# marsermd/DeepestScatter

Measured on AMD Instinct MI355X. Metric: Msamples/s (rays x spp) at 512^3 vol, 1024^2 frame; HBM GB/s vs roofline, higher is better.
Workload: dtype f32

## Files before the change

### deepestscatter_amd/cloudtrace.py

```python
from __future__ import annotations

import ctypes as C
from dataclasses import dataclass
from pathlib import Path

import numpy as np

from . import _lib
from ._lib import (CT_BUF_DENSITY, CT_BUF_FRAME, CT_BUF_INSCATTER, CT_BUF_M2, CT_BUF_MEAN, CT_BUF_SCREEN,
                   CtCounters, CtFetchCounters, CtScene, check)

MIE_FILE = Path(__file__).resolve().parent / "data" / "mie_raw.f32"

LIGHT_DIRECTIONS = {
    "Front": (-0.586, -0.766, -0.271),
    "Side": (-0.03, -0.25, 0.8),
    "Back": (0.586, -0.766, -0.271),
}


def load_mie_raw() -> tuple[np.ndarray, np.ndarray]:
    raw = np.fromfile(MIE_FILE, dtype="<f4")
    if raw.size != 8192:
        raise RuntimeError(f"{MIE_FILE} is corrupt")
# ... 545 lines not shown
        c = CtCounters()
        check(self.L.ct_counters(self.h, C.byref(c)), self.h)
        return c.as_dict()

    def fetch_counters(self) -> dict:
        c = CtFetchCounters()
        check(self.L.ct_fetch_counters(self.h, C.byref(c)), self.h)
        return c.as_dict()

    def debug_invariants(self) -> dict:
        out = np.zeros(8, np.uint64)
        check(self.L.ct_debug_invariants(self.h, _p(out)), self.h)
        names = ["armed", "checks", "violations", "samples_without_alpha_1", "dealt", "resumed", "written", "suspended"]
        return {n: int(v) for n, v in zip(names, out)}

    def debug_memory(self) -> dict:
        out = np.zeros(8, np.uint64)
        check(self.L.ct_debug_memory(self.h, _p(out)), self.h)
        names = ["raw_texture", "density_bricks", "inscatter_bricks", "march_bricks_dense", "march_bricks_stored", "sparse",
                 "row_table", "coarse_clearance"]
        return {n: int(v) for n, v in zip(names, out)}

    def delta_grid(self) -> dict:
        out = np.zeros(8, np.uint32)
        check(self.L.ct_debug_delta_grid(self.h, _p(out)), self.h)
        return {"cell": int(out[0]), "stored": tuple(int(v) for v in out[1:4]), "origin": tuple(int(v) for v in out[4:7]),
                "nee": int(out[7] & 0xff), "interior": bool(out[7] & 0x100)}

    def march_meta(self) -> dict:
        geom = np.zeros(8, np.uint32)
        check(self.L.ct_debug_march_meta(self.h, _p(geom), C.c_void_p(), 0), self.h)
        d = {"radius": int(geom[0]), "bias_x": int(geom[1]), "bias": int(geom[2]),
             "bricks": tuple(int(v) for v in geom[3:6]), "sparse": bool(geom[6]), "meta": None}
        if not d["sparse"]:
            gx, gy, gz = d["bricks"]
            meta = np.zeros((gz * 4, gy * 4, gx), np.uint8)
            check(self.L.ct_debug_march_meta(self.h, _p(geom), _p(meta), meta.size), self.h)
            d["meta"] = meta
        return d

    LAYOUTS = ("density_bricks", "shadow_bricks", "march_bricks", "march_rows", "march_coarse", "twin_bricks", "majorant_cells",
               "majorant_codes", "mip_pyramid")

    def layout(self, which) -> tuple[np.ndarray, dict]:
        which = self.LAYOUTS.index(which) if isinstance(which, str) else int(which)
        geom, n = np.zeros(16, np.uint32), C.c_size_t(0)
        check(self.L.ct_debug_layout(self.h, which, _p(geom), C.c_void_p(), 0, C.byref(n)), self.h)
        g = [int(v) for v in geom]
        raw = np.zeros(n.value, np.uint8)
        check(self.L.ct_debug_layout(self.h, which, _p(geom), _p(raw), raw.size, C.byref(n)), self.h)
        if which in (_lib.CT_LAYOUT_DENSITY_BRICKS, _lib.CT_LAYOUT_SHADOW_BRICKS, _lib.CT_LAYOUT_TWIN_BRICKS):
            d = {"bias": g[0], "bricks": tuple(g[1:4])}
            return raw.reshape(g[3], g[2], g[1], 128), d
        if which == _lib.CT_LAYOUT_MARCH_BRICKS:
            d = {"bias_x": g[0], "bias": g[1], "bricks": tuple(g[2:5]), "sparse": bool(g[5])}
            return (raw.reshape(-1, 128) if d["sparse"] else raw.reshape(g[4], g[3], g[2], 128)), d
        if which == _lib.CT_LAYOUT_MARCH_ROWS:
            return raw.view(np.uint32).reshape(g[1], g[0], 2), {"rows": (g[0], g[1])}
        if which == _lib.CT_LAYOUT_MARCH_COARSE:
            return raw.reshape(g[3], g[2], g[1]), {"shift": g[0], "cells": tuple(g[1:4]), "bias": g[4]}
        if which == _lib.CT_LAYOUT_MIP_PYRAMID:
            return raw, {"levels": g[0], "dims": tuple(g[1:4])}
        d = {"cell": g[0], "div": g[1], "stored": tuple(g[2:5]), "origin": tuple(g[5:8]), "virtual": tuple(g[8:11]), "bias": g[11]}
        return raw.reshape(g[4], g[3], g[2]), d

    def kernel_time(self):
        a, b, n = C.c_double(0), C.c_double(0), C.c_uint64(0)
        check(self.L.ct_kernel_time(self.h, C.byref(a), C.byref(b), C.byref(n)), self.h)
        return float(a.value), float(b.value), int(n.value)

    def set_stream(self, hip_stream: int | None):
        check(self.L.ct_set_stream(self.h, C.c_void_p(hip_stream) if hip_stream else None), self.h)

    def debug_stats(self) -> dict:
        out = np.zeros(64, np.uint64)
        check(self.L.ct_debug_stats(self.h, _p(out)), self.h)
        names = ["regen_phases", "regen_lanes", "march_phases", "march_lanes", "scatter_phases", "scatter_lanes",
                 "fetched_steps", "fetched_zero_cells", "skipped_steps", "zero_cells_nonfree_brick",
                 "zero_cells_free_brick_d1", "skip_loop_wave_iterations", "nee_footprints_reused", "waves",
                 "stolen_jobs", "max_scheduler_visits_of_a_wave"]
        d = {n: int(v) for n, v in zip(names, out)}
        d["wave_end_hist_5ms"] = [int(v) for v in out[16:40]]
        d["wave_end_minus_drained_hist_0p5ms"] = [int(v) for v in out[40:64]]
        ex = np.zeros(73, np.uint64)
        check(self.L.ct_debug_stats_ex(self.h, _p(ex), 73), self.h)
        d["march_fetch_same_line_as_lanes_previous"] = int(ex[68])
        d["march_fetch_line_shared_with_a_lower_lane"] = int(ex[69])
        d["nee_lookups_skipped_shadow_zero"] = int(ex[72])
        d["raw"] = [int(v) for v in out]
        d["watchdog"] = int(out[63])
        return d

    def debug_suspended(self) -> int:
        n = C.c_uint64(0)
        check(self.L.ct_debug_suspended(self.h, C.byref(n)), self.h)
        return int(n.value)

    def debug_math_selftest(self, which: int) -> dict:
        out = np.zeros(3, np.uint64)
        check(self.L.ct_debug_math_selftest(self.h, which, _p(out)), self.h)
        return {"tested": int(out[0]), "mismatches": int(out[1]), "first_bad_bits": int(out[2])}

    def debug_cdf_inversion(self, first_u24: int, count: int) -> np.ndarray:
        out = np.empty(count, np.uint32)
        check(self.L.ct_debug_cdf_inversion(self.h, first_u24, count, _p(out)), self.h)
        return out


class TracerGroup:

    def __init__(self, density: np.ndarray, devices, params: SceneParams | None = None, **kw):
        self.L = _lib.load()
        self.params = params or SceneParams(**kw)
        s, keep = make_scene(density, self.params)
        self.width, self.height = self.params.width, self.params.height
        dev = np.asarray(list(devices), np.int32)
        g = C.c_void_p()
        rc = self.L.ct_group_create(C.byref(s), _p(dev), len(dev), C.byref(g))
        del keep
        if rc != _lib.CT_OK:
            msg = self.L.ct_group_last_error(None)
            raise _lib.CloudTraceError(rc, msg.decode("utf-8", "replace") if msg else "")
        self.g = g

    def _check(self, rc):
        if rc != _lib.CT_OK:
            msg = self.L.ct_group_last_error(self.g)
            raise _lib.CloudTraceError(rc, msg.decode("utf-8", "replace") if msg else "")

    def close(self):
        if getattr(self, "g", None):
            for net in list(getattr(self, "_networks", ())):
                net.close()
            self.L.ct_group_destroy(self.g)
            self.g = None

    def __enter__(self):
        return self

    def __exit__(self, *exc):
        self.close()

    def __del__(self):
        try:
            self.close()
        except Exception:
            pass

    def set_camera(self, eye, U, V, W):
        a = [np.asarray(v, np.float32) for v in (eye, U, V, W)]
        self._check(self.L.ct_group_set_camera(self.g, *[_p(v) for v in a]))

    def set_light(self, direction, color=None, intensity: float = 1e6):
        d, c = _light_args(direction, color)
        self._check(self.L.ct_group_set_light(self.g, _p(d) if d is not None else None, _p(c) if c is not None else None, intensity))

    def render_accumulate(self, first_subframe_id: int, count: int):
        self._check(self.L.ct_group_render_accumulate(self.g, first_subframe_id, count))

    def network(self, module_or_weights, width: int | None = None, aux: int | None = None, head_layers: int | None = None):
        return GroupNetwork(self, module_or_weights, width, aux, head_layers)

    def network_render_accumulate(self, net, first_subframe_id: int, count: int, transform="linear", rgb_scale=(1.0, 1.0, 1.0),
                                  band_pixels: int = 0, direct: bool = False):
        p = CloudTracer._network_render_params(transform, rgb_scale, band_pixels, direct)
        self._check(self.L.ct_group_network_render_accumulate(self.g, net.gn if net is not None else None, C.byref(p),
                                                              first_subframe_id & 0xFFFFFFFF, count))

    def reset(self):
        self._check(self.L.ct_group_reset(self.g))

# ... 72 lines not shown
```

### deepestscatter_amd/csrc/ct_api.cpp

```cpp
#include <algorithm>
#include <array>
#include <atomic>
#include <chrono>
#include <climits>
#include <cmath>
#include <cstdarg>
#include <cstdio>
#include <cstdlib>
#include <cstring>
#include <new>
#include <string>
#include <utility>
#include <map>
#include <vector>

#include "../../include/cloudtrace.h"
#include "ct_handle.hpp"

static thread_local std::string g_create_error;

int ct::fail(CtHandle h, int code, const char *fmt, ...)
{
    char buf[512];
    va_list ap;
// ... 436 lines not shown
{
    const uint32_t n[3] = { nx, ny, nz };
    uint32_t faces = 0;
    for (uint32_t f = 0; f < 6; f++) {
        const uint32_t axis = f / 2, u_axis = (axis + 1) % 3, v_axis = (axis + 2) % 3;
        uint32_t c[3];
        c[axis] = (f & 1) ? n[axis] - 1 : 0;
        bool zero = true;
        for (c[v_axis] = 0; zero && c[v_axis] < n[v_axis]; c[v_axis]++) {
            for (c[u_axis] = 0; zero && c[u_axis] < n[u_axis]; c[u_axis]++) {
                zero = t[((size_t)c[2] * ny + c[1]) * nx + c[0]] == 0;
            }
        }
        faces |= (zero ? 1u : 0u) << f;
    }
    return faces;
}

struct MarchStorage {
    bool sparse;
    bool vmm;
    bool pad_rows;
    bool experimental;
};

static MarchStorage march_storage(const CtScene *s, const Knob &sparse_knob)
{
    bool sparse = (s->flags & CT_FLAG_SPARSE_BRICKS) != 0, vmm = (s->flags & CT_FLAG_VMM_BRICKS) != 0, pad_only = false, no_pad = false;
    if (const char *env = sparse_knob.get()) {
        const int v = atoi(env);
        sparse = v == 1;
        vmm = v == 2 || v == 4;
        pad_only = v == 3;
        no_pad = v == 4;
    }
    const bool march = s->estimator == CT_EST_MARCH;
    vmm = vmm && march;
    return { sparse && march, vmm && !sparse, (vmm && !no_pad) || pad_only, vmm || pad_only };
}

static int open_device(const CtScene *s, CtHandle h)
{
    int ndev = 0;
    if (hipGetDeviceCount(&ndev) != hipSuccess || ndev <= 0) {
        return fail(h, CT_E_NODEVICE, "no HIP device visible (libcloudtrace has no CPU fallback)");
    }
    if (s->device < 0 || s->device >= ndev) {
        return fail(h, CT_E_INVAL, "device %d out of range (0..%d)", s->device, ndev - 1);
    }
    HIPCHK(h, hipSetDevice(s->device));
    (void)hipGetLastError();
    HIPCHK(h, hipStreamCreateWithFlags(&h->own_stream, hipStreamNonBlocking));
    h->stream = h->own_stream;
    for (auto &e : h->ev) {
        HIPCHK(h, hipEventCreate(&e));
    }
    return CT_OK;
}

static int choose_schedule(const CtScene *s, CtHandle h)
{
    const CtTuning &t = h->tune;
    DevScene &d = h->dev;
    const bool delta = s->estimator == CT_EST_DELTA, big = beyond_caches(s);
    h->shape = persistent_shape(s->device, delta, knob_int(t.BLOCKS_PER_CU, INT_MIN, INT_MAX, 0));
    h->debug_invariants = knob_flag(t.DEBUG_INVARIANTS, h->debug_invariants);
    h->shape.stats = t.STATS.get() != nullptr || h->debug_invariants;
    h->exchange = delta ? knob_int(t.EXCHANGE, 0, 2, 0) : 0;
#ifdef CT_EXPERIMENTS
    if (h->exchange && (s->flags & CT_FLAG_TEX_FIXED8)) {
        return fail(h, CT_E_INVAL, "CT_EXCHANGE has no CT_FLAG_TEX_FIXED8 kernels");
    }
    if (h->exchange) {
        h->xshape = h->exchange == 2 ? wave_exchange_shape(s->device) : exchange_shape(s->device);
        h->xshape.stats = h->shape.stats;
    }
#else
    if (h->exchange) {
        return fail(h, CT_E_INVAL, "CT_EXCHANGE needs the experiments build (python -m deepestscatter_amd.build --variant exp; "
                                   "CT_LIBRARY=libcloudtrace_exp.so)");
    }
#endif
    d.march_burst = (uint32_t)knob_int(t.MARCH_BURST, 1, 1024, delta ? 2 : 8);
    d.burst_scatter = (uint32_t)knob_int(t.BURST_SCATTER, 1, 65, delta || big ? 48 : 40);
    d.burst_idle = (uint32_t)knob_int(t.BURST_IDLE, 1, 65, 32);
    d.burst_march_min = (uint32_t)knob_int(t.BURST_MARCH_MIN, 1, 64, 1);
    d.tail_burst = (uint32_t)knob_int(t.TAIL_BURST, 1, 1024, 8);
    d.regen_min = (uint32_t)knob_int(t.REGEN_MIN, 1, 64, delta ? 4 : big ? 16 : 8);
    d.scatter_min = (uint32_t)knob_int(t.SCATTER_MIN, 1, 64, delta ? 12 : 1);
    d.scatter_num = 0;
    d.scatter_den = 1;
    if (const char *e = t.SCATTER_RATIO.get()) {
        unsigned a = 1, b = 1;
        if (sscanf(e, "%u/%u", &a, &b) == 2 && b > 0 && a < 1000 && b < 1000) {
            d.scatter_num = a;
            d.scatter_den = b;
        }
    }
    d.hint_period = 64;
    if (const char *e = t.HINT_PERIOD.get()) {
        const int v = atoi(e);
        d.hint_period = (v > 0 && (v & (v - 1)) == 0) ? (uint32_t)v : 0u;
    }
    if (delta) {
        d.delta_nee = (uint32_t)knob_int(t.DELTA_NEE, 0, 2, big ? 2 : 1);
        h->job_work = 48.f;
    }
    h->queues_enabled = knob_flag(t.XCD_QUEUES, big);
    h->regions = (uint32_t)knob_int(t.XCD_REGIONS, 1, 65536, (int)h->regions);
    if (const char *e = t.SHARED_DEPTH.get()) {
        h->shared_depth = (float)atof(e);
    }
    h->job_max = (uint32_t)knob_int(t.JOB_MAX, 1, 4096, (int)h->job_max);
    if (const char *e = t.JOB_WORK.get()) {
        h->job_work = (float)std::max(1.0, atof(e));
    }
    h->no_advance = knob_flag(t.NO_ADVANCE, h->no_advance);
    h->point_order = knob_flag(t.POINT_ORDER, h->point_order);
    h->continuation = knob_flag(t.CONTINUATION, h->continuation) && !h->exchange;
    h->chunk_interleave = knob_flag(t.CHUNK_INTERLEAVE, h->chunk_interleave);
    if (const char *e = t.TILE_ORDER.get()) {
        h->tile_hilbert = strcmp(e, "hilbert") == 0;
    }
    h->chunk_morton = knob_flag(t.CHUNK_MORTON, h->chunk_morton);
    h->serpentine = knob_flag(t.SERPENTINE, h->serpentine);
    h->hand_on_jobs = knob_flag(t.HAND_ON_JOBS, h->hand_on_jobs);
    h->max_age_override = knob_int(t.MAX_AGE, 0, CtHandle_::kMaxRegions - 1, h->max_age_override);
    h->ahead = (uint32_t)knob_int(t.RENDER_AHEAD, 0, 65535, (int)h->ahead);
    return CT_OK;
}

static void light_uniforms(const CtScene *s, DevScene &d)
{
    float l[3] = { s->light_direction[0], s->light_direction[1], s->light_direction[2] };
    if (!(s->flags & CT_FLAG_LIGHT_NORMALIZED)) {
        v3_normalize_twice(s->light_direction, l);
    }
    d.nlx = -l[0];
    d.nly = -l[1];
    d.nlz = -l[2];
    d.lr = s->light_color[0] * s->light_intensity;
    d.lg = s->light_color[1] * s->light_intensity;
    d.lb = s->light_color[2] * s->light_intensity;
}

static void scene_uniforms(const CtScene *s, DevScene &d)
{
    const uint32_t nx = s->dims[0], ny = s->dims[1], nz = s->dims[2];
    const float fx = (float)nx, fy = (float)ny, fz = (float)nz;
    const float maxs = fmaxf(fmaxf(fx, fy), fz);
    d.nx = (int32_t)nx;
    d.ny = (int32_t)ny;
    d.nz = (int32_t)nz;
    d.bx = fx / maxs;
    d.by = fy / maxs;
    d.bz = fz / maxs;
    d.hx = d.bx + 0.01f;
    d.hy = d.by + 0.01f;
    d.hz = d.bz + 0.01f;
    d.tsx = maxs / fx;
    d.tsy = maxs / fy;
    d.tsz = maxs / fz;
    d.sx = (maxs / fx) * fx;
    d.sy = (maxs / fy) * fy;
    d.sz = (maxs / fz) * fz;
    d.density_multiplier = s->cloud_size_m / s->mean_free_path_m;
    d.sample_step = s->sample_step;
// ... 2597 lines not shown
```

### deepestscatter_amd/csrc/ct_internal.hpp

```cpp
#pragma once

#include <hip/hip_runtime.h>
#include <stdint.h>

#include "ct_device.hpp"

namespace ct {

constexpr int kTile = 8;
constexpr int kCounterCount = 9;
constexpr int kStatCount = 73;
constexpr int kContWords = 16;
constexpr int kContWordsDelta = 32;
constexpr int kLeftWords = 8;
constexpr int kQueueFlag = 32;
constexpr int kQueueDone = 16;
constexpr int kQueueWords = 64;
constexpr int kQueues = 8;

struct BatchArgs {
    float4 *frames;
    uint32_t frame_stride;
    const float4 *primary;
    const float4 *advance;
    const uint32_t *pixels;
    const float4 *start;
    const uint32_t *group_rank;
    uint32_t rank_base;
    const uint32_t *job_group;
    const uint32_t *job_sub;
    uint2 *cost;
    uint32_t n_jobs;
    uint32_t q_begin[kQueues + 2];
    uint32_t reverse;
    uint32_t first_subframe;
    uint32_t S;
    uint32_t *queue;
    const uint32_t *cont_in;
    const uint32_t *cont_in_count;
    uint32_t *cont_cursor;
    uint32_t *cont_out;
    uint32_t *cont_out_count;
    uint32_t cont_capacity;
    uint32_t max_age;
    unsigned long long *cont_total;
    const uint32_t *left_in;
    const uint32_t *left_in_count;
    uint32_t *left_cursor;
    uint32_t *left_out;
    uint32_t *left_out_count;
    uint32_t left_capacity;
    uint32_t out_offset;
    unsigned long long *counters;
    unsigned long long *stats;
    unsigned long long *timeline;
    uint32_t *touched_density, *touched_shadow;
};

struct LaunchShape {
    int blocks;
    int threads;
    bool stats;
    uint32_t pool_slots = 0;
    uint32_t scatter_waves = 0;
    bool wide = false;
};

inline void split_queues_evenly(BatchArgs &ba)
{
    for (int x = 0; x <= kQueues; x++) {
        ba.q_begin[x] = (uint32_t)(((uint64_t)ba.n_jobs * (uint32_t)x) / kQueues);
    }
    ba.q_begin[kQueues + 1] = ba.n_jobs;
}

#ifndef CT_SHARD_SHIFT
#define CT_SHARD_SHIFT 0
#endif
__host__ __device__ inline uint32_t tile_owner(uint32_t tx, uint32_t ty, uint32_t shard_count)
{
    return shard_count <= 1 ? 0u : ((tx >> CT_SHARD_SHIFT) + 3u * (ty >> CT_SHARD_SHIFT)) % shard_count;
}

hipError_t launch_build_bricks(const uint8_t *texels, int nx, int ny, int nz, int bias, int gx, int gy, int gz,
                               uint8_t *bricks, hipStream_t stream);
hipError_t launch_build_twin_bricks(const uint8_t *density, const uint8_t *shadow, int nx, int ny, int nz, int bias, int gx, int gy, int gz,
                                    uint8_t *bricks, hipStream_t stream);
hipError_t launch_build_dist(const uint8_t *texels, int nx, int ny, int nz, int bias, int gx, int gy, int gz,
                             uint8_t *dist, uint8_t *scratch, uint8_t *majorant, hipStream_t stream);
hipError_t launch_majorant_cells(const uint8_t *texels, int nx, int ny, int nz, int bias, int cell, const int origin[3], int gx, int gy, int gz,
                                 uint8_t *out, uint8_t *out_codes, hipStream_t stream);
hipError_t launch_brick_meta(const uint8_t *dist, const uint8_t *majorant, int nx, int ny, int nz, int bias, int gx,
                             int gy, int gz, uint8_t *bricks, hipStream_t stream);
hipError_t launch_build_mbricks(const uint8_t *texels, int nx, int ny, int nz, int bias_x, int bias, int gx, int gy,
// ... 148 lines not shown
```

### deepestscatter_amd/csrc/ct_kernels.hip

```cpp
#include <algorithm>
#include <cstdlib>

#include "ct_internal.hpp"

namespace ct {

__global__ void build_bricks_kernel(const uint8_t *__restrict__ t, int nx, int ny, int nz, int bias,
                                    uint8_t *__restrict__ bricks, int gx, int gy, int gz)
{
    const int64_t total = (int64_t)gx * gy * gz * 128;
    for (int64_t i = (int64_t)blockIdx.x * blockDim.x + threadIdx.x; i < total; i += (int64_t)gridDim.x * blockDim.x) {
        const int64_t b = i >> 7;
        const int o = (int)(i & 127);
        uint8_t v = 0;
        if (o < 125) {
            const int lx = o % 5, ly = (o / 5) % 5, lz = o / 25;
            const int x = (int)(b % gx) * 4 + lx - bias;
            const int y = (int)((b / gx) % gy) * 4 + ly - bias;
            const int z = (int)(b / ((int64_t)gx * gy)) * 4 + lz - bias;
            const int xc = min(max(x, 0), nx - 1), yc = min(max(y, 0), ny - 1), zc = min(max(z, 0), nz - 1);
            v = t[((size_t)zc * ny + yc) * nx + xc];
        }
        bricks[i] = v;
    }
// ... 858 lines not shown
                                        uint32_t &nee_key, uint2 &nee_cell, bool &reused, bool zero = false)
{
    NeeLoads n;
    const float cos_light = dot3(mk3(sc.nlx, sc.nly, sc.nlz), dir);
    const float u = (cos_light + 1) / 2;
    const float x = fmaf(u, (float)kMieN, -0.5f);
    const int32_t i = (int32_t)floorf(x);
    const int32_t j = min(max(i, 0), kMieN - 2);
    float2 pair;
#if CT_MARCH_PHASE_LDS == 2
    LdsFloat *table = chopped ? (LdsFloat *)lds.chopped : (LdsFloat *)lds.mie;
    pair = make_float2(table[j], table[j + 1]);
#elif CT_MARCH_PHASE_LDS == 1
    LdsFloat *table = (LdsFloat *)lds.chopped;
    pair = make_float2(table[j], table[j + 1]);
    if (!chopped) {
        GlobalFloat *first = (GlobalFloat *)(sc.mie + j);
        pair = make_float2(first[0], first[1]);
    }
#else
    if (chopped) {
        pair = make_float2(lds.chopped[j], lds.chopped[j + 1]);
    } else {
        __builtin_memcpy(&pair, sc.mie + j, sizeof pair);
    }
#endif
    n.a = (i > kMieN - 2) ? pair.y : pair.x;
    n.b = (i < 0) ? pair.x : pair.y;
    n.w = tex_weight<FIXED8>(x);
    n.cell = fetch_cell_cached<WIDE>(sc, sc.ibricks, pos, nee_key, nee_cell, reused, zero);
    return n;
}

template <bool FIXED8>
CT_DEV f3 in_scattering_finish(const DevScene &sc, const NeeLoads &n, f3 pos)
{
    const float phase = fmaf(n.w, n.b - n.a, n.a);
    const float ins = filter_at<FIXED8>(sc, n.cell, pos);
    f3 l = scale3(mk3(sc.lr, sc.lg, sc.lb), ins);
    l = scale3(l, phase);
    return scale3(l, sc.sun_ratio);
}

enum : int { ST_IDLE = 0, ST_MARCH = 1, ST_BOUNCE = 2 };

#ifndef CT_MARCH_FLAT_ZERO
#define CT_MARCH_FLAT_ZERO 1
#endif
#ifndef CT_MARCH_FLAT_EXIT
#define CT_MARCH_FLAT_EXIT 1
#endif
#ifndef CT_MARCH_FUSE
#define CT_MARCH_FUSE 1
#endif
constexpr bool MARCH_FUSE = CT_MARCH_FUSE != 0;
#ifndef CT_MARCH_NEE_SKIP
#define CT_MARCH_NEE_SKIP 1
#endif

CT_DEV float inv_max_advance(const DevScene &sc, f3 stepv)
{
    const float m = fmaxf(fmaxf(fabsf(stepv.x) * sc.sx, fabsf(stepv.y) * sc.sy), fabsf(stepv.z) * sc.sz);
    return __builtin_amdgcn_rcpf(fmaxf(m, 1e-20f));
}


CT_DEV int skip_steps(uint32_t c, float inv_maxd)
{
    return (int)(((float)c - 0.03125f) * inv_maxd);
}

CT_DEV void replay_steps(f3 &pos, f3 stepv, int n)
{
    int i = 0;
    for (; i + 8 <= n; i += 8) {
#pragma unroll
        for (int k = 0; k < 8; k++) {
            pos = add3(pos, stepv);
        }
    }
    for (; i < n; i++) {
        pos = add3(pos, stepv);
    }
}

template <bool FIXED8, bool SPARSE = false>
__global__ __launch_bounds__(256) void inscatter_kernel(DevScene sc, uint8_t *__restrict__ out, uint32_t zero_faces)
{
    const int64_t total = (int64_t)sc.nx * sc.ny * sc.nz;
    const int64_t i = (int64_t)blockIdx.x * blockDim.x + threadIdx.x;
    if (i >= total) {
        return;
    }
    const int x = (int)(i % sc.nx), y = (int)((i / sc.nx) % sc.ny), z = (int)(i / ((int64_t)sc.nx * sc.ny));
    const float max_size = (float)max(max(sc.nx, sc.ny), sc.nz);
    const float tsx = max_size / (float)sc.nx, tsy = max_size / (float)sc.ny, tsz = max_size / (float)sc.nz;
    const float min_scale = fminf(fminf(tsx, tsy), tsz);
    const float inv_min_scale = 1.0f / min_scale;
    f3 p = mk3((float)x / max_size, (float)y / max_size, (float)z / max_size);
    p = scale3(p, inv_min_scale);
    const f3 step_to_light = scale3(normalize3(mk3(sc.nlx, sc.nly, sc.nlz)), sc.sample_step);
    const int step_count = (int)(1 / sc.sample_step);
    float transmittance = 1;
    int s = 0;
    bool done = false;
    if (sc.mbricks != nullptr && (SPARSE || sc.m_rows == nullptr)) {
        const float inv_maxd = inv_max_advance(sc, step_to_light);
        while (s < step_count && in_box(sc, p)) {
            uint32_t meta;
            const uint2 cell = fetch_cell_m<SPARSE>(sc, p, meta);
            if ((cell.x | cell.y) != 0u) {
                const float density = filter_at<FIXED8>(sc, cell, p) * sc.density_multiplier;
                const float extinction = density * sc.sample_step;
                transmittance *= ct_expf(-extinction);
                if (transmittance * 255.f < 1.f) {
                    done = true;
                    break;
                }
            }
            p = add3(p, step_to_light);
            s += 1;
            const uint32_t clear = meta & 0x3fu;
            if (clear != 0u) {
                const int n = min(skip_steps(clear, inv_maxd), step_count - s);
                replay_steps(p, step_to_light, n);
                s += n;
            }
        }
    }
    for (; !done && s < step_count; s++) {
        const float tx = fmaf(p.x, sc.sx, -0.5f), ty = fmaf(p.y, sc.sy, -0.5f), tz = fmaf(p.z, sc.sz, -0.5f);
        const bool gone = ((zero_faces & 1u) && tx < 0.0f && step_to_light.x <= 0.0f) ||
                          ((zero_faces & 2u) && tx >= (float)(sc.nx - 1) && step_to_light.x >= 0.0f) ||
                          ((zero_faces & 4u) && ty < 0.0f && step_to_light.y <= 0.0f) ||
                          ((zero_faces & 8u) && ty >= (float)(sc.ny - 1) && step_to_light.y >= 0.0f) ||
                          ((zero_faces & 16u) && tz < 0.0f && step_to_light.z <= 0.0f) ||
                          ((zero_faces & 32u) && tz >= (float)(sc.nz - 1) && step_to_light.z >= 0.0f);
        if (gone) {
            break;
        }
        const float density = tex3_clamped<FIXED8>(sc, sc.dbricks, p) * sc.density_multiplier;
        const float extinction = density * sc.sample_step;
        transmittance *= ct_expf(-extinction);
        p = add3(p, step_to_light);
        if (transmittance * 255.f < 1.f) {
            break;
        }
    }
    out[i] = (uint8_t)(transmittance * 255.f);
}

hipError_t launch_inscatter(const DevScene &sc, uint8_t *out, uint32_t zero_faces, hipStream_t stream)
{
    const int64_t total = (int64_t)sc.nx * sc.ny * sc.nz;
    const int threads = 256;
    const int64_t blocks = (total + threads - 1) / threads;
    const dim3 grid((unsigned)blocks), block(threads);
    if (sc.mbricks != nullptr && sc.m_rows != nullptr) {
        if (sc.tex_fixed8) {
            hipLaunchKernelGGL((inscatter_kernel<true, true>), grid, block, 0, stream, sc, out, zero_faces);
        } else {
            hipLaunchKernelGGL((inscatter_kernel<false, true>), grid, block, 0, stream, sc, out, zero_faces);
        }
    } else if (sc.tex_fixed8) {
        hipLaunchKernelGGL(inscatter_kernel<true>, grid, block, 0, stream, sc, out, zero_faces);
    } else {
// ... 42 lines not shown
        }
    }
    advance[p] = make_float4(start.x, start.y, start.z, __uint_as_float(start_bits));
}

hipError_t launch_primary_advance(const DevScene &sc, const float4 *primary, float4 *advance, hipStream_t stream)
{
    const dim3 grid((sc.width + 31) / 32, (sc.height + 7) / 8), block(256);
    if (sc.m_rows) {
        hipLaunchKernelGGL(primary_advance_kernel<true>, grid, block, 0, stream, sc, primary, advance);
    } else {
        hipLaunchKernelGGL(primary_advance_kernel<false>, grid, block, 0, stream, sc, primary, advance);
    }
    return hipGetLastError();
}

__global__ __launch_bounds__(256) void start_records_kernel(DevScene sc, const uint32_t *__restrict__ pixels, uint32_t slots,
                                                            const float4 *__restrict__ primary, const float4 *__restrict__ advance,
                                                            float4 *__restrict__ start)
{
    const uint32_t i = blockIdx.x * 256u + threadIdx.x;
    if (i >= slots) {
        return;
    }
    const uint32_t pixel = pixels[i];
    float4 r0 = make_float4(0.f, 0.f, 0.f, __uint_as_float(0xc0000000u)), r1 = make_float4(0.f, 0.f, 0.f, 0.f);
    if (pixel != 0xffffffffu) {
        const float4 p0 = primary[2 * (size_t)pixel];
        r1 = primary[2 * (size_t)pixel + 1];
        const bool go = p0.w != 0.f && in_box(sc, mk3(p0.x, p0.y, p0.z));
        uint32_t bits = go ? 0u : 0x80000000u;
        r0 = p0;
        if (go && advance) {
            r0 = advance[pixel];
            bits |= __float_as_uint(r0.w) & 0x3fffffffu;
        }
        r0.w = __uint_as_float(bits);
    }
    start[2 * (size_t)i] = r0;
    start[2 * (size_t)i + 1] = r1;
}

hipError_t launch_start_records(const DevScene &sc, const uint32_t *pixels, uint32_t slots, const float4 *primary,
                                const float4 *advance, float4 *start, hipStream_t stream)
{
    hipLaunchKernelGGL(start_records_kernel, dim3((slots + 255u) / 256u), dim3(256), 0, stream, sc, pixels, slots, primary, advance, start);
    return hipGetLastError();
}

template <int MODE, bool STATS, bool SPARSE, bool COST = true, bool FIXED8 = false, bool WIDE = false>
__global__ __launch_bounds__(kMarchThreads) __attribute__((amdgpu_waves_per_eu(6))) void render_persistent_kernel(DevScene sc, BatchArgs ba)
{
    __shared__ MieLdsFull lds;
    load_tables(sc, lds);

    const uint32_t lane = threadIdx.x & 63u;
#ifdef CT_DIAG_TIMELINE
    if (ba.timeline && lane == 0u) {
        ba.timeline[4u * (blockIdx.x * (blockDim.x >> 6) + (threadIdx.x >> 6))] = wall_clock64();
    }
#endif
    f3 pos = mk3(0, 0, 0), dir = mk3(0, 0, 1), stepv = mk3(0, 0, 0), rad = mk3(0, 0, 0);
    uint32_t seed = 0, depth = 0, out_idx = 0;
    uint32_t work = 0;
    float xi = 0, T = 1;
    uint32_t dfree = 0;
    float inv_maxd = 0;
    int state = ST_IDLE;

    JobState job{ 0, 0, 0, 0, 0, 0 };
    bool left_done = false;
    uint32_t q_cur = (uint32_t)kQueues, q_tried = 0;
    bool drained = false;
    uint32_t c_dl = 0, c_il = 0, c_cap = 0;
    uint32_t w_fetch = 0, w_nee = 0;
    uint32_t iv_dealt = 0, iv_written = 0, iv_resumed = 0, iv_suspended = 0;
    uint32_t nee_key = 0xffffffffu;
    uint2 nee_cell = make_uint2(0u, 0u);
    uint32_t st_regen = 0, st_regen_l = 0, st_march = 0, st_march_l = 0, st_scat = 0, st_scat_l = 0;
    uint32_t st_fetch = 0, st_zero = 0, st_skip = 0, st_zero_d0 = 0, st_zero_d1 = 0, st_skip_iters = 0, st_stolen = 0, st_iters = 0, st_first = 0;
    uint32_t st_hit2 = 0, st_hit3 = 0, st_h2 = 0xffffffffu, st_h3 = 0xffffffffu;
    uint32_t st_same_line = 0, st_dup_line = 0, st_prev_line = 0xffffffffu;
    uint32_t st_nee_zero = 0;

    uint32_t age = 0;
    if (ba.cont_in) {
        const uint32_t total = __builtin_amdgcn_readfirstlane(*ba.cont_in_count);
        uint32_t base = 0;
        if (lane == 0) {
            base = atomicAdd(ba.cont_cursor, 64u);
        }
        base = __builtin_amdgcn_readfirstlane(base);
        if (base + lane < total) {
            const uint4 *e = (const uint4 *)(ba.cont_in + (size_t)(base + lane) * kContWords);
            const uint4 w0 = e[0], w1 = e[1], w2 = e[2], w3 = e[3];
            pos = mk3(__uint_as_float(w0.x), __uint_as_float(w0.y), __uint_as_float(w0.z));
            dir = mk3(__uint_as_float(w0.w), __uint_as_float(w1.x), __uint_as_float(w1.y));
            rad = mk3(__uint_as_float(w1.z), __uint_as_float(w1.w), __uint_as_float(w2.x));
            seed = w2.y;
            out_idx = w2.z;
            xi = __uint_as_float(w2.w);
            T = __uint_as_float(w3.x);
            inv_maxd = __uint_as_float(w3.y);
            depth = w3.z & 0xffffu;
            dfree = (w3.z >> 16) & 0xffu;
            state = (int)(w3.z >> 24);
            stepv = scale3(dir, sc.sample_step);
            age = w3.w;
            if (STATS) {
                iv_resumed += 1;
            }
        }
    }
    const bool may_suspend = ba.cont_out != nullptr;
    const bool single_queue = ba.q_begin[1] == ba.n_jobs;

    const unsigned long long t_start = STATS ? wall_clock64() : 0ull;
    unsigned long long t_drained = 0;
#ifdef CT_DIAG_TIMELINE
    bool tl_marked = false;
#endif
    uint32_t visit = 0;
    for (;;) {
        visit += 1;
        if (may_suspend && single_queue && !drained && sc.hint_period != 0u && (visit & (sc.hint_period - 1u)) == 0u) {
            const uint32_t empty = __builtin_amdgcn_readfirstlane(__atomic_load_n(ba.queue + kQueueFlag, __ATOMIC_RELAXED));
            if (empty != 0u) {
                if (job.next != job.end && ba.left_out && job.age < ba.max_age && hand_on_job(ba, lane, job)) {
                    job.next = job.end;
                }
                if (job.next == job.end) {
                    drained = true;
                }
            }
        }
#ifdef CT_DIAG_TIMELINE
        if (ba.timeline && drained && !tl_marked) {
            tl_marked = true;
            const uint32_t live = (uint32_t)__builtin_popcountll(__builtin_amdgcn_ballot_w64(state != ST_IDLE));
            const uint32_t old = (uint32_t)__builtin_popcountll(__builtin_amdgcn_ballot_w64(state != ST_IDLE && age >= ba.max_age));
            if (lane == 0u) {
                unsigned long long *tl = ba.timeline + 4u * (blockIdx.x * (blockDim.x >> 6) + (threadIdx.x >> 6));
                tl[2] = wall_clock64();
                tl[3] = live | (old << 8) | ((job.next != job.end ? 1u : 0u) << 16);
            }
        }
#endif
        if (STATS) {
            st_iters += 1;
            if (drained && t_drained == 0) {
                t_drained = wall_clock64();
            }
        }
        const uint64_t idle = __builtin_amdgcn_ballot_w64(state == ST_IDLE);
        const uint32_t n_idle = (uint32_t)__builtin_popcountll(idle);
        if ((n_idle >= sc.regen_min || n_idle == 64u) && !(drained && job.next == job.end)) {
            if (job.next == job.end && !take_leftover(ba, lane, left_done, job)) {
                uint32_t j = 0;
                if (!take_job(ba, lane, q_cur, q_tried, j)) {
                    drained = true;
                } else {
                    if (STATS) {
                        st_stolen += (q_tried != 0u) ? 1u : 0u;
                    }
                    const uint32_t sub = __builtin_amdgcn_readfirstlane(ba.job_sub[j]);
                    const uint32_t s0 = sub & 0xffffu;
// ... 110 lines not shown
                st_scat += 1;
                st_scat_l += nb;
            }
            bool nee_fetched = false;
            if (state == ST_BOUNCE) {
                bool nee_zero = false;
                {
                    const float lg = logf_above_one(div_(xi, T));
                    const float inv = rcp_moderate(inv_maxd);
                    pos = sub3(pos, scale3(scale3(dir, lg), inv));
                    nee_zero = CT_MARCH_NEE_SKIP != 0 && (dfree & 0x40u) != 0u && lg * inv <= sc.nee_reach;
                }
                if ((dfree & 0x80u) != 0u || in_box(sc, pos)) {
                    const bool chopped = (MODE == 1) ? true : (MODE == 0 ? (depth != 1) : false);
                    bool nee_reused = false;
                    const uint32_t st_key_before = nee_key;
                    NeeLoads nee;
                    if (CT_MARCH_NEE_SKIP == 1) {
                        if (!nee_zero) {
                            nee = in_scattering_issue_lds<FIXED8, WIDE>(sc, lds, pos, dir, chopped, nee_key, nee_cell, nee_reused);
                        }
                    } else {
                        nee = in_scattering_issue_lds<FIXED8, WIDE>(sc, lds, pos, dir, chopped, nee_key, nee_cell, nee_reused, nee_zero);
                    }
                    if (STATS) {
                        st_nee_zero += nee_zero ? 1u : 0u;
                        nee_reused = nee_reused || nee_zero;
                    }
                    if (STATS && !nee_reused) {
                        st_hit2 += (nee_key == st_h2) ? 1u : 0u;
                        st_hit3 += (nee_key != st_h2 && nee_key == st_h3) ? 1u : 0u;
                        st_h3 = st_h2;
                        st_h2 = st_key_before;
                    }
                    nee_fetched = !nee_reused && !nee_zero;
                    if (STATS) {
                        st_first += nee_reused ? 1u : 0u;
                        if (ba.touched_shadow && !nee_reused) {
                            const uint32_t line = (uint32_t)(apron_offset_in_grid(sc, pos) >> 7);
                            atomicOr(&ba.touched_shadow[line >> 5], 1u << (line & 31u));
                        }
                    }
                    c_il += 1;
                    if (COST) {
                        work += 4u;
                    }
                    bool go = (MODE != 2);
                    if (go) {
                        dir = new_direction(lds.cdf, lds.guide, seed, dir);
                        depth++;
                        if (depth == sc.max_depth) {
                            c_cap += 1;
                            go = false;
                        }
                    }
                    if (CT_MARCH_NEE_SKIP != 1 || !nee_zero) {
                        rad = add3(rad, in_scattering_finish<FIXED8>(sc, nee, pos));
                    }
                    if (go) {
                        xi = u24_to_float(lcg24(seed));
                        T = 1;
                        stepv = scale3(dir, sc.sample_step);
                        inv_maxd = inv_max_advance(sc, stepv);
                        dfree = 0;
                        state = ST_MARCH;
                    } else {
                        finished = true;
                    }
                } else {
                    finished = true;
                }
            }
            w_nee += (uint32_t)__builtin_popcountll(__builtin_amdgcn_ballot_w64(nee_fetched));
        }
        bool track = !do_scatter;
        uint32_t nm_track = nm;
        if (do_scatter && MARCH_FUSE) {
            nm_track = (uint32_t)__builtin_popcountll(__builtin_amdgcn_ballot_w64(state == ST_MARCH));
            track = nm_track != 0u;
        }
        if (track) {
            if (STATS) {
                st_march += 1;
                st_march_l += nm_track;
            }
            w_fetch += nm_track;
            uint32_t burst = drained ? sc.tail_burst : sc.march_burst;
            for (;;) {
            if (state == ST_MARCH) {
                if (dfree != 0u) {
                    const int n = skip_steps(dfree, inv_maxd);
                    replay_steps(pos, stepv, n);
                    c_dl += (uint32_t)n;
                    if (STATS) {
                        st_skip += (uint32_t)n;
                        int wmax = n;
#pragma unroll
                        for (int off = 32; off > 0; off >>= 1) {
                            wmax = max(wmax, __shfl_xor(wmax, off));
                        }
                        st_skip_iters += (lane_rank(__builtin_amdgcn_ballot_w64(true)) == 0u) ? (uint32_t)wmax : 0u;
                    }
                }
                pos = add3(pos, stepv);
                uint32_t meta;
                const uint2 cell = fetch_cell_m<SPARSE, WIDE>(sc, pos, meta);
                dfree = meta & 0x3fu;
                c_dl += 1;
                if (COST) {
                    work += 1u;
                }
                if (STATS) {
                    st_fetch += 1;
                    {
                        const float fx = fmaf(pos.x, sc.sx, -0.5f), fy = fmaf(pos.y, sc.sy, -0.5f), fz = fmaf(pos.z, sc.sz, -0.5f);
                        const uint32_t lx = (uint32_t)(floor_to_int(fx) + sc.m_bias_x), ly = (uint32_t)(floor_to_int(fy) + sc.brick_bias),
                                       lz = (uint32_t)(floor_to_int(fz) + sc.brick_bias);
                        const uint32_t line = __umul24(lz >> 2, (uint32_t)sc.m_gxy) + __umul24(ly >> 2, (uint32_t)sc.m_gx) + (__umul24(lx, 43691u) >> 17);
                        st_same_line += (line == st_prev_line) ? 1u : 0u;
                        st_prev_line = line;
                        if (ba.touched_density && !SPARSE) {
                            atomicOr(&ba.touched_density[line >> 5], 1u << (line & 31u));
                        }
                        const uint64_t act = __builtin_amdgcn_ballot_w64(true);
                        bool dup = false;
                        for (uint32_t i = 0; i < 64u; i++) {
                            const uint32_t other = (uint32_t)__builtin_amdgcn_readlane((int)line, (int)i);
                            dup = dup || (((act >> i) & 1ull) != 0ull && i < lane && other == line);
                        }
                        st_dup_line += dup ? 1u : 0u;
                    }
                    st_zero += ((cell.x | cell.y) == 0u) ? 1u : 0u;
                    st_zero_d0 += ((cell.x | cell.y) == 0u && dfree == 0u) ? 1u : 0u;
                    st_zero_d1 += ((cell.x | cell.y) == 0u && dfree == 1u) ? 1u : 0u;
                }
                bool collided = false;
                if (CT_MARCH_FLAT_ZERO || (cell.x | cell.y) != 0u) {
                    const float density = filter_at<FIXED8>(sc, cell, pos) * sc.density_multiplier;
                    const float extinction = density * sc.sample_step;
                    T *= expf_inrange(-extinction);
                    if (xi > T) {
                        collided = true;
                        inv_maxd = density;
                    }
                }
#if CT_MARCH_FLAT_EXIT
                state = collided ? ST_BOUNCE : state;
                dfree = collided ? (meta & 0xc0u) : dfree;
                if (!collided & ((meta & 0x80u) == 0u) & !in_box_flat(sc, pos)) {
#else
                if (collided) {
                    state = ST_BOUNCE;
                    dfree = meta & 0xc0u;
                } else if ((meta & 0x80u) == 0u && !in_box(sc, pos)) {
#endif
                    ba.frames[out_idx] = make_float4(rad.x, rad.y, rad.z, 1.f);
                    if (STATS) {
                        iv_written += 1;
                    }
                    if (COST && ba.cost) {
                        ba.cost[out_idx - ba.out_offset] = make_uint2(work, depth);
                    }
                    state = ST_IDLE;
                }
            }
            if (--burst == 0u) {
                break;
            }
            const uint32_t m_now = (uint32_t)__builtin_popcountll(__builtin_amdgcn_ballot_w64(state == ST_MARCH));
            const uint32_t b_now = (uint32_t)__builtin_popcountll(__builtin_amdgcn_ballot_w64(state == ST_BOUNCE));
            if (drained) {
                if (m_now == 0u || 2u * b_now >= m_now + b_now) {
                    break;
                }
            } else if (m_now < sc.burst_march_min || b_now >= sc.burst_scatter || 64u - m_now - b_now >= sc.burst_idle) {
                break;
            }
            w_fetch += m_now;
            if (STATS) {
                st_march += 1;
                st_march_l += m_now;
            }
            }
        }
        if (finished) {
            ba.frames[out_idx] = make_float4(rad.x, rad.y, rad.z, 1.f);
            if (STATS) {
                iv_written += 1;
            }
            if (COST && ba.cost) {
                ba.cost[out_idx - ba.out_offset] = make_uint2(work, depth);
            }
            state = ST_IDLE;
        }
        if (may_suspend && drained && job.next == job.end) {
            const bool mine = state != ST_IDLE && age < ba.max_age;
            const uint64_t live = __builtin_amdgcn_ballot_w64(mine);
            if (live != 0ull) {
                const uint32_t n = (uint32_t)__builtin_popcountll(live);
                uint32_t base = 0;
                if (lane == (uint32_t)__builtin_ctzll(live)) {
                    base = atomicAdd(ba.cont_out_count, n);
                    if (base + n > ba.cont_capacity) {
                        atomicSub(ba.cont_out_count, n);
                        base = 0xffffffffu;
                    } else if (ba.cont_total) {
                        atomicAdd(ba.cont_total, (unsigned long long)n);
                    }
                }
                base = __builtin_amdgcn_readlane(base, __builtin_ctzll(live));
                if (mine && base != 0xffffffffu) {
                    uint4 *e = (uint4 *)(ba.cont_out + (size_t)(base + lane_rank(live)) * kContWords);
                    e[0] = make_uint4(__float_as_uint(pos.x), __float_as_uint(pos.y), __float_as_uint(pos.z), __float_as_uint(dir.x));
                    e[1] = make_uint4(__float_as_uint(dir.y), __float_as_uint(dir.z), __float_as_uint(rad.x), __float_as_uint(rad.y));
                    e[2] = make_uint4(__float_as_uint(rad.z), seed, out_idx, __float_as_uint(xi));
                    e[3] = make_uint4(__float_as_uint(T), __float_as_uint(inv_maxd), depth | (dfree << 16) | ((uint32_t)state << 24), age + 1u);
                    state = ST_IDLE;
                    if (STATS) {
                        iv_suspended += 1;
                    }
                }
            }
        }
    }

#ifdef CT_DIAG_TIMELINE
    if (ba.timeline && lane == 0u) {
        ba.timeline[4u * (blockIdx.x * (blockDim.x >> 6) + (threadIdx.x >> 6)) + 1u] = wall_clock64();
    }
#endif
    const uint32_t vals[3] = { wave_sum(c_dl), wave_sum(c_il), wave_sum(c_cap) };
    if (STATS) {
        uint32_t sv[16] = { st_fetch, st_zero, st_skip, st_zero_d0, st_zero_d1, st_skip_iters, st_first,
                            iv_dealt, iv_resumed, iv_written, iv_suspended, st_same_line, st_dup_line, st_hit2, st_hit3, st_nee_zero };
#pragma unroll
        for (int i = 0; i < 16; i++) {
            sv[i] = wave_sum(sv[i]);
        }
        if (lane == 0) {
            atomicAdd(&ba.stats[0], (unsigned long long)st_regen);
            atomicAdd(&ba.stats[1], (unsigned long long)st_regen_l);
            atomicAdd(&ba.stats[2], (unsigned long long)st_march);
            atomicAdd(&ba.stats[3], (unsigned long long)st_march_l);
            atomicAdd(&ba.stats[4], (unsigned long long)st_scat);
            atomicAdd(&ba.stats[5], (unsigned long long)st_scat_l);
            atomicAdd(&ba.stats[6], (unsigned long long)sv[0]);
            atomicAdd(&ba.stats[7], (unsigned long long)sv[1]);
            atomicAdd(&ba.stats[8], (unsigned long long)sv[2]);
            atomicAdd(&ba.stats[9], (unsigned long long)sv[3]);
            atomicAdd(&ba.stats[10], (unsigned long long)sv[4]);
            atomicAdd(&ba.stats[11], (unsigned long long)sv[5]);
            atomicAdd(&ba.stats[12], (unsigned long long)sv[6]);
            atomicAdd(&ba.stats[13], 1ull);
            atomicAdd(&ba.stats[14], (unsigned long long)st_stolen);
            atomicMax(&ba.stats[15], (unsigned long long)st_iters);
            const unsigned long long t_end = wall_clock64();
#ifdef CT_STATS_FINE
            atomicAdd(&ba.stats[16 + min((unsigned long long)23, (t_end - t_start) / 25000ull)], 1ull);
            atomicAdd(&ba.stats[40 + min((unsigned long long)23, (t_end - (t_drained ? t_drained : t_end)) / 5000ull)], 1ull);
#else
            atomicAdd(&ba.stats[16 + min((unsigned long long)23, (t_end - t_start) / 500000ull)], 1ull);
            atomicAdd(&ba.stats[40 + min((unsigned long long)23, (t_end - (t_drained ? t_drained : t_end)) / 50000ull)], 1ull);
#endif
            atomicAdd(&ba.stats[64], (unsigned long long)sv[7]);
            atomicAdd(&ba.stats[65], (unsigned long long)sv[8]);
            atomicAdd(&ba.stats[66], (unsigned long long)sv[9]);
            atomicAdd(&ba.stats[67], (unsigned long long)sv[10]);
            atomicAdd(&ba.stats[68], (unsigned long long)sv[11]);
            atomicAdd(&ba.stats[69], (unsigned long long)sv[12]);
            atomicAdd(&ba.stats[70], (unsigned long long)sv[13]);
            atomicAdd(&ba.stats[71], (unsigned long long)sv[14]);
            atomicAdd(&ba.stats[72], (unsigned long long)sv[15]);
        }
    }
    flush_counters(ba, lane, vals[0], vals[1], vals[2], w_fetch, w_nee);
}

__global__ void mip_level_kernel(const uint8_t *__restrict__ prev, int px, int py, int pz, uint8_t *__restrict__ cur,
                                 int cx, int cy, int cz)
{
    const int64_t total = (int64_t)cx * cy * cz;
    for (int64_t i = (int64_t)blockIdx.x * blockDim.x + threadIdx.x; i < total; i += (int64_t)gridDim.x * blockDim.x) {
        const int x = (int)(i % cx), y = (int)((i / cx) % cy), z = (int)(i / ((int64_t)cx * cy));
        uint32_t acc = 0;
#pragma unroll
        for (int d = 0; d < 8; d++) {
            const int sx = 2 * x + (d & 1), sy = 2 * y + ((d >> 1) & 1), sz = 2 * z + (d >> 2);
            if (sx < px && sy < py && sz < pz) {
                acc += prev[((size_t)sz * py + sy) * px + sx];
            }
        }
        cur[i] = (uint8_t)(acc / 8u);
    }
}

hipError_t launch_mip_level(const uint8_t *prev, int px, int py, int pz, uint8_t *cur, int cx, int cy, int cz,
                            hipStream_t stream)
{
    const int64_t total = (int64_t)cx * cy * cz;
    const int blocks = (int)std::min<int64_t>((total + 255) / 256, 65536);
    hipLaunchKernelGGL(mip_level_kernel, dim3(blocks), dim3(256), 0, stream, prev, px, py, pz, cur, cx, cy, cz);
    return hipGetLastError();
}

template <bool FIXED8>
CT_DEV float tex3_level(const DevScene &sc, const MipPyramid &mp, uint32_t l, f3 p)
{
    const int32_t nx = mp.nx[l], ny = mp.ny[l], nz = mp.nz[l];
    const float x = fmaf(p.x, sc.tsx * (float)nx, -0.5f), y = fmaf(p.y, sc.tsy * (float)ny, -0.5f),
                z = fmaf(p.z, sc.tsz * (float)nz, -0.5f);
    const float flx = floorf(x), fly = floorf(y), flz = floorf(z);
    const float wx = tex_weight<FIXED8>(x), wy = tex_weight<FIXED8>(y), wz = tex_weight<FIXED8>(z);
    const int32_t ix = (int32_t)flx, iy = (int32_t)fly, iz = (int32_t)flz;
    const int32_t x0 = min(max(ix, 0), nx - 1), x1 = min(max(ix + 1, 0), nx - 1);
    const int32_t y0 = min(max(iy, 0), ny - 1), y1 = min(max(iy + 1, 0), ny - 1);
    const int32_t z0 = min(max(iz, 0), nz - 1), z1 = min(max(iz + 1, 0), nz - 1);
    const uint8_t *b = mp.base + mp.offset[l];
    const size_t sy_ = (size_t)nx, sz_ = (size_t)nx * (size_t)ny;
    uint2 c;
    c.x = (uint32_t)b[z0 * sz_ + y0 * sy_ + x0] | ((uint32_t)b[z0 * sz_ + y0 * sy_ + x1] << 8) |
          ((uint32_t)b[z0 * sz_ + y1 * sy_ + x0] << 16) | ((uint32_t)b[z0 * sz_ + y1 * sy_ + x1] << 24);
    c.y = (uint32_t)b[z1 * sz_ + y0 * sy_ + x0] | ((uint32_t)b[z1 * sz_ + y0 * sy_ + x1] << 8) |
          ((uint32_t)b[z1 * sz_ + y1 * sy_ + x0] << 16) | ((uint32_t)b[z1 * sz_ + y1 * sy_ + x1] << 24);
    return filter_cell(c, wx, wy, wz);
}

template <bool FIXED8>
__global__ __launch_bounds__(256) void descriptor_kernel(DevScene sc, MipPyramid mp, const float *__restrict__ positions,
                                                         const float *__restrict__ directions, uint32_t count,
                                                         float level0, float voxel_m, float cloud_size_m,
                                                         uint8_t *__restrict__ out)
{
    const uint32_t layer = blockIdx.x % 10u, i = blockIdx.x / 10u;
    const uint32_t sample = threadIdx.x;
    if (i >= count || sample >= 225u) {
        return;
    }
    const f3 world = mk3(positions[3 * (size_t)i], positions[3 * (size_t)i + 1], positions[3 * (size_t)i + 2]);
    const f3 view = mk3(directions[3 * (size_t)i], directions[3 * (size_t)i + 1], directions[3 * (size_t)i + 2]);
    const f3 ez = normalize3(mk3(sc.nlx, sc.nly, sc.nlz));
    const f3 ex = normalize3(cross3(ez, view));
    const f3 ey = cross3(ex, ez);
    const f3 origin = add3(world, scale3(mk3(sc.bx, sc.by, sc.bz), 0.5f));
    float scale = 0.5f / sc.density_multiplier;
    float lod = level0;
    for (uint32_t l = 0; l < layer; l++) {
        scale *= 2;
        lod += 1;
    }
    const float mip_voxel = ct_powf(2.0f, lod) * voxel_m / cloud_size_m;
    const int x = (int)(sample % 5u) - 2, y = (int)((sample / 5u) % 5u) - 2, z = (int)(sample / 25u) - 2;
    const f3 dir = add3(add3(scale3(ex, (float)x), scale3(ey, (float)y)), scale3(ez, (float)z));
    const f3 pos = add3(origin, scale3(dir, scale));
    uint8_t *const dst = out + ((size_t)i * 10u + layer) * 225u + sample;
    if (!(isfinite(pos.x) && isfinite(pos.y) && isfinite(pos.z))) {
// ... 2120 lines not shown
```

Measured before the change: 3759.

## Bound free-space skip replay per march iteration to reduce wave divergence

```diff
diff --git a/deepestscatter_amd/cloudtrace.py b/deepestscatter_amd/cloudtrace.py
--- a/deepestscatter_amd/cloudtrace.py
+++ b/deepestscatter_amd/cloudtrace.py
@@ -651,11 +651,13 @@
         d = {n: int(v) for n, v in zip(names, out)}
         d["wave_end_hist_5ms"] = [int(v) for v in out[16:40]]
         d["wave_end_minus_drained_hist_0p5ms"] = [int(v) for v in out[40:64]]
-        ex = np.zeros(73, np.uint64)
-        check(self.L.ct_debug_stats_ex(self.h, _p(ex), 73), self.h)
+        ex = np.zeros(75, np.uint64)
+        check(self.L.ct_debug_stats_ex(self.h, _p(ex), 75), self.h)
         d["march_fetch_same_line_as_lanes_previous"] = int(ex[68])
         d["march_fetch_line_shared_with_a_lower_lane"] = int(ex[69])
         d["nee_lookups_skipped_shadow_zero"] = int(ex[72])
+        d["free_space_skips"] = int(ex[73])
+        d["replay_lane_steps"] = int(ex[74])
         d["raw"] = [int(v) for v in out]
         d["watchdog"] = int(out[63])
         return d
diff --git a/deepestscatter_amd/csrc/ct_api.cpp b/deepestscatter_amd/csrc/ct_api.cpp
--- a/deepestscatter_amd/csrc/ct_api.cpp
+++ b/deepestscatter_amd/csrc/ct_api.cpp
@@ -542,7 +542,7 @@
     }
 #endif
     d.march_burst = (uint32_t)knob_int(t.MARCH_BURST, 1, 1024, delta ? 2 : 8);
-    d.burst_scatter = (uint32_t)knob_int(t.BURST_SCATTER, 1, 65, delta || big ? 48 : 40);
+    d.burst_scatter = (uint32_t)knob_int(t.BURST_SCATTER, 1, 65, delta || big ? 48 : 32);
     d.burst_idle = (uint32_t)knob_int(t.BURST_IDLE, 1, 65, 32);
     d.burst_march_min = (uint32_t)knob_int(t.BURST_MARCH_MIN, 1, 64, 1);
     d.tail_burst = (uint32_t)knob_int(t.TAIL_BURST, 1, 1024, 8);
diff --git a/deepestscatter_amd/csrc/ct_internal.hpp b/deepestscatter_amd/csrc/ct_internal.hpp
--- a/deepestscatter_amd/csrc/ct_internal.hpp
+++ b/deepestscatter_amd/csrc/ct_internal.hpp
@@ -9,7 +9,7 @@
 
 constexpr int kTile = 8;
 constexpr int kCounterCount = 9;
-constexpr int kStatCount = 73;
+constexpr int kStatCount = 75;
 constexpr int kContWords = 16;
 constexpr int kContWordsDelta = 32;
 constexpr int kLeftWords = 8;
diff --git a/deepestscatter_amd/csrc/ct_kernels.hip b/deepestscatter_amd/csrc/ct_kernels.hip
--- a/deepestscatter_amd/csrc/ct_kernels.hip
+++ b/deepestscatter_amd/csrc/ct_kernels.hip
@@ -964,6 +964,22 @@
     for (; i < n; i++) {
         pos = add3(pos, stepv);
     }
+}
+
+#ifndef CT_MARCH_REPLAY_MAX
+#define CT_MARCH_REPLAY_MAX 4
+#endif
+
+CT_DEV uint32_t replay_bounded(f3 &pos, f3 stepv, uint32_t owed)
+{
+#pragma unroll
+    for (uint32_t k = 0; k < (uint32_t)CT_MARCH_REPLAY_MAX; k++) {
+        if (k >= owed) {
+            break;
+        }
+        pos = add3(pos, stepv);
+    }
+    return owed - min(owed, (uint32_t)CT_MARCH_REPLAY_MAX);
 }
 
 template <bool FIXED8, bool SPARSE = false>
@@ -1172,6 +1188,7 @@
     uint32_t st_hit2 = 0, st_hit3 = 0, st_h2 = 0xffffffffu, st_h3 = 0xffffffffu;
     uint32_t st_same_line = 0, st_dup_line = 0, st_prev_line = 0xffffffffu;
     uint32_t st_nee_zero = 0;
+    uint32_t st_skips = 0, st_replay_l = 0;
 
     uint32_t age = 0;
     if (ba.cont_in) {
@@ -1448,11 +1465,40 @@
         if (track) {
             if (STATS) {
                 st_march += 1;
-                st_march_l += nm_track;
-            }
+                st_march_l += CT_MARCH_REPLAY_MAX == 0 ? nm_track : 0u;
+            }
+#if CT_MARCH_REPLAY_MAX == 0
             w_fetch += nm_track;
+#endif
             uint32_t burst = drained ? sc.tail_burst : sc.march_burst;
             for (;;) {
+#if CT_MARCH_REPLAY_MAX != 0
+            if (state == ST_MARCH && dfree != 0u) {
+                uint32_t owed = dfree >> 8;
+                if ((dfree & 0xffu) != 0u) {
+                    owed = (uint32_t)skip_steps(dfree & 0xffu, inv_maxd);
+                    c_dl += owed;
+                    if (STATS) {
+                        st_skip += owed;
+                        st_skips += owed != 0u ? 1u : 0u;
+                    }
+                }
+                if (STATS) {
+                    st_replay_l += owed != 0u ? 1u : 0u;
+                    st_skip_iters += (lane_rank(__builtin_amdgcn_ballot_w64(true)) == 0u) ? 1u : 0u;
+                }
+                dfree = replay_bounded(pos, stepv, owed) << 8;
+            }
+            const bool steps = state == ST_MARCH && dfree == 0u;
+            {
+                const uint32_t n_steps = (uint32_t)__builtin_popcountll(__builtin_amdgcn_ballot_w64(steps));
+                w_fetch += n_steps;
+                if (STATS) {
+                    st_march_l += n_steps;
+                }
+            }
+            if (steps) {
+#else
             if (state == ST_MARCH) {
                 if (dfree != 0u) {
                     const int n = skip_steps(dfree, inv_maxd);
@@ -1466,8 +1512,11 @@
                             wmax = max(wmax, __shfl_xor(wmax, off));
                         }
                         st_skip_iters += (lane_rank(__builtin_amdgcn_ballot_w64(true)) == 0u) ? (uint32_t)wmax : 0u;
+                        st_skips += n > 0 ? 1u : 0u;
+                        st_replay_l += n > 0 ? 1u : 0u;
                     }
                 }
+#endif
                 pos = add3(pos, stepv);
                 uint32_t meta;
                 const uint2 cell = fetch_cell_m<SPARSE, WIDE>(sc, pos, meta);
@@ -1542,10 +1591,12 @@
             } else if (m_now < sc.burst_march_min || b_now >= sc.burst_scatter || 64u - m_now - b_now >= sc.burst_idle) {
                 break;
             }
+#if CT_MARCH_REPLAY_MAX == 0
             w_fetch += m_now;
+#endif
             if (STATS) {
                 st_march += 1;
-                st_march_l += m_now;
+                st_march_l += CT_MARCH_REPLAY_MAX == 0 ? m_now : 0u;
             }
             }
         }
@@ -1577,6 +1628,12 @@
                 base = __builtin_amdgcn_readlane(base, __builtin_ctzll(live));
                 if (mine && base != 0xffffffffu) {
                     uint4 *e = (uint4 *)(ba.cont_out + (size_t)(base + lane_rank(live)) * kContWords);
+#if CT_MARCH_REPLAY_MAX != 0
+                    for (uint32_t owed = dfree >> 8; owed != 0u; owed--) {
+                        pos = add3(pos, stepv);
+                    }
+                    dfree &= 0xffu;
+#endif
                     e[0] = make_uint4(__float_as_uint(pos.x), __float_as_uint(pos.y), __float_as_uint(pos.z), __float_as_uint(dir.x));
                     e[1] = make_uint4(__float_as_uint(dir.y), __float_as_uint(dir.z), __float_as_uint(rad.x), __float_as_uint(rad.y));
                     e[2] = make_uint4(__float_as_uint(rad.z), seed, out_idx, __float_as_uint(xi));
@@ -1597,10 +1654,11 @@
 #endif
     const uint32_t vals[3] = { wave_sum(c_dl), wave_sum(c_il), wave_sum(c_cap) };
     if (STATS) {
-        uint32_t sv[16] = { st_fetch, st_zero, st_skip, st_zero_d0, st_zero_d1, st_skip_iters, st_first,
-                            iv_dealt, iv_resumed, iv_written, iv_suspended, st_same_line, st_dup_line, st_hit2, st_hit3, st_nee_zero };
+        uint32_t sv[18] = { st_fetch, st_zero, st_skip, st_zero_d0, st_zero_d1, st_skip_iters, st_first,
+                            iv_dealt, iv_resumed, iv_written, iv_suspended, st_same_line, st_dup_line, st_hit2, st_hit3, st_nee_zero,
+                            st_skips, st_replay_l };
 #pragma unroll
-        for (int i = 0; i < 16; i++) {
+        for (int i = 0; i < 18; i++) {
             sv[i] = wave_sum(sv[i]);
         }
         if (lane == 0) {
@@ -1637,6 +1695,8 @@
             atomicAdd(&ba.stats[70], (unsigned long long)sv[13]);
             atomicAdd(&ba.stats[71], (unsigned long long)sv[14]);
             atomicAdd(&ba.stats[72], (unsigned long long)sv[15]);
+            atomicAdd(&ba.stats[73], (unsigned long long)sv[16]);
+            atomicAdd(&ba.stats[74], (unsigned long long)sv[17]);
         }
     }
     flush_counters(ba, lane, vals[0], vals[1], vals[2], w_fetch, w_nee);
```

Result: faster. 3884, median of 6 (+3.3%).
